# darchr/DLRM.jl

Hardware: NVIDIA B200
Metric: dlrm_train_samples_per_sec (higher is better)
Workload: dtype f32 (3xTF32 interaction forward)

## Files before the change

dlrm_jl_b200/_lib.py:

```python
from __future__ import annotations

import ctypes as C
import os
from typing import Optional

HERE = os.path.dirname(os.path.abspath(__file__))
LIB_PATH = os.path.join(HERE, "lib", "libdlrm_b200.so")

OK, EINVAL, ECUDA, ENOMEM, EOOB, ESTATE, ENCCL = 0, 1, 2, 3, 4, 5, 6
_STATUS_NAMES = {EINVAL: "DLRMB_EINVAL", ECUDA: "DLRMB_ECUDA", ENOMEM: "DLRMB_ENOMEM",
                 EOOB: "DLRMB_EOOB", ESTATE: "DLRMB_ESTATE", ENCCL: "DLRMB_ENCCL"}


class DLRMB200Error(RuntimeError):
    def __init__(self, status: int, message: str):
        super().__init__(f"{_STATUS_NAMES.get(status, status)}: {message}")
        self.status = status


_i32, _i64, _f32, _vp = C.c_int32, C.c_int64, C.c_float, C.c_void_p
_idx_args = [_vp, _i32, _i32, _i32, _i32]
_idx_mp_args = [_vp, _i32, _i32, _i32, C.POINTER(_i32)]

SIGNATURES = {
    "dlrmb_abi_version": (_i32, []),
    "dlrmb_last_error": (C.c_char_p, []),
    "dlrmb_launch_count": (_i64, []),
    "dlrmb_set_option": (_i32, [C.c_char_p, _i64]),
    "dlrmb_get_option": (_i32, [C.c_char_p, C.POINTER(_i64)]),
    "dlrmb_clock_buffer_bytes": (_i64, []),
    "dlrmb_clock_kernels": (_i32, []),
    "dlrmb_clock_enable": (_i32, [_vp]),
    "dlrmb_tables_create": (_i32, [_i32, _i32, C.POINTER(_i64), _i32, _i64, C.POINTER(_vp)]),
    "dlrmb_tables_create_ex": (_i32, [_i32, _i32, C.POINTER(_i64), _i32, _i64, _i32, C.POINTER(_vp)]),
    "dlrmb_tables_elem_bytes": (_i32, [_vp]),
    "dlrmb_tables_reserve": (_i32, [_vp, _i64]),
    "dlrmb_tables_destroy": (_i32, [_vp]),
    "dlrmb_tables_info": (_i32, [_vp, C.POINTER(_i32), C.POINTER(_i32), C.POINTER(_i64), C.POINTER(_i64)]),
    "dlrmb_tables_upload": (_i32, [_vp, _i32, _vp]),
    "dlrmb_tables_download": (_i32, [_vp, _i32, _vp]),
    "dlrmb_tables_device_ptr": (_i32, [_vp, _i32, C.POINTER(_vp)]),
    "dlrmb_tables_init_uniform": (_i32, [_vp, C.c_uint64, _vp]),
    "dlrmb_tables_sync": (_i32, [_vp]),
    "dlrmb_embedding_fwd": (_i32, [_vp, *_idx_args, _vp, _i32, _i32, _vp]),
    "dlrmb_embedding_fwd_sort": (_i32, [_vp, *_idx_args, _vp, _i32, _i32, _vp]),
    "dlrmb_interaction_fwd": (_i32, [_i32, _vp, _vp, _i32, _i32, _i32, _i32, _vp, _vp]),
    "dlrmb_interaction_bwd": (_i32, [_i32, _vp, _vp, _i32, _i32, _i32, _i32, _vp, _vp, _vp]),
    "dlrmb_embedding_sort": (_i32, [_vp, *_idx_args, _vp]),
    "dlrmb_embedding_update_sorted": (_i32, [_vp, _vp, _i32, _i32, _f32, _vp]),
    "dlrmb_embedding_bwd_sgd": (_i32, [_vp, *_idx_args, _vp, _i32, _i32, _f32, _vp]),
    "dlrmb_sort_dedup_export": (_i32, [_vp, _i32, _vp, _vp, _vp, C.POINTER(_i32)]),
    "dlrmb_check_indices": (_i32, [_vp, *_idx_args, _i32]),
    "dlrmb_bce_sigmoid_fwd_bwd": (_i32, [_i32, _vp, _vp, _i32, _vp, _vp, _vp, _vp, _vp]),
    "dlrmb_xbuf_create": (_i32, [_i32, _i64, C.POINTER(_vp)]),
    "dlrmb_xbuf_destroy": (_i32, [_vp]),
    "dlrmb_xbuf_ptr": (_i32, [_vp, C.POINTER(_vp)]),
    "dlrmb_xbuf_ipc_handle": (_i32, [_vp, _vp]),
    "dlrmb_xbuf_open": (_i32, [_i32, _vp, C.POINTER(_vp)]),
    "dlrmb_xbuf_close": (_i32, [_i32, _vp]),
    "dlrmb_tables_set_slot_map": (_i32, [_vp, C.POINTER(_i32)]),
    "dlrmb_embedding_fwd_p2p": (_i32, [_vp, *_idx_args, C.POINTER(_vp), _i32, _i32, _i32, _vp]),
    "dlrmb_embedding_fwd_p2p_sort": (_i32, [_vp, *_idx_args, C.POINTER(_vp), _i32, _i32, _i32, _vp]),
    "dlrmb_embedding_fwd_p2p_mp": (_i32, [_vp, *_idx_mp_args, C.POINTER(_vp), _i32, _i32, _i32, _vp]),
    "dlrmb_embedding_fwd_p2p_sort_mp": (_i32, [_vp, *_idx_mp_args, C.POINTER(_vp), _i32, _i32, _i32, _vp]),
    "dlrmb_peer_barrier": (_i32, [_i32, C.POINTER(_vp), _i32, _i32, _i32, _vp, _vp]),
    "dlrmb_peer_barrier_flag_bytes": (_i64, []),
    "dlrmb_peer_barrier_state_bytes": (_i64, []),
    "dlrmb_peer_allreduce_f32": (_i32, [_i32, C.POINTER(_vp), C.POINTER(_vp), _i32, _i32, _i32, _vp, _vp, _i64, _vp]),
    "dlrmb_indices_scatter_p2p": (_i32, [_i32, _vp, _i32, _i32, _i32, _i32, _vp, _i32, _vp]),
    "dlrmb_indices_scatter_p2p_mp": (_i32, [_i32, _vp, _i32, _i32, _i32, C.POINTER(_i32), _vp, _i32, _vp]),
    "dlrmb_interaction_has_warp_path": (_i32, [_i32, _i32]),
    "dlrmb_dense_fwd_bias_act": (_i32, [_i32, _vp, _vp, _i32, _i32, _i32, _vp]),
    "dlrmb_dense_bwd_scratch_floats": (_i64, [_i32]),
    "dlrmb_dense_bwd_act_bias": (_i32, [_i32, _vp, _vp, _i32, _i32, _vp, _vp, _vp, _vp]),
    "dlrmb_interaction_bwd_scatter": (_i32, [_i32, _vp, _vp, _i32, _i32, _i32, _i32, _vp, _i64, _vp, _vp]),
    "dlrmb_interaction_bwd_dx": (_i32, [_i32, _vp, _vp, _i32, _i32, _i32, _i32, _vp, _vp]),
    "dlrmb_dac_unpack": (_i32, [_i32, _vp, _i32, _vp, _vp, _vp, _vp]),
    "dlrmb_shard_plan": (_i32, [_i32, C.POINTER(_i64), _i32, C.POINTER(_i32)]),
    "dlrmb_shard_plan_mp": (_i32, [_i32, C.POINTER(_i64), C.POINTER(_i32), _i32, C.POINTER(_i32)]),
    "dlrmb_comm_unique_id": (_i32, [_vp]),
    "dlrmb_comm_create": (_i32, [_i32, _vp, _i32, _i32, C.POINTER(_vp)]),
    "dlrmb_comm_destroy": (_i32, [_vp]),
    "dlrmb_comm_info": (_i32, [_vp, C.POINTER(_i32), C.POINTER(_i32)]),
    "dlrmb_comm_a2a_indices": (_i32, [_vp, C.POINTER(_i32), _i32, _vp, _i32, _i32, _i32, _vp, _vp]),
    "dlrmb_comm_a2a_indices_mp": (_i32, [_vp, C.POINTER(_i32), _i32, _vp, _i32, _i32, C.POINTER(_i32), _vp, _vp]),
    "dlrmb_comm_a2a_fwd": (_i32, [_vp, C.POINTER(_i32), _i32, _vp, _i32, _i32, _vp, _vp]),
    "dlrmb_comm_a2a_bwd": (_i32, [_vp, C.POINTER(_i32), _i32, _vp, _i32, _i32, _vp, _vp]),
    "dlrmb_comm_allreduce_f32": (_i32, [_vp, _vp, _i64, _vp]),
    "dlrmb_comm_allgather": (_i32, [_vp, _vp, _vp, _i64, _vp]),
    "dlrmb_embedding_fwd_host": (_i32, [_vp, *_idx_args, _vp, _i32, _i32]),
    "dlrmb_interaction_fwd_host": (_i32, [_vp, _vp, _vp, _i32, _i32, _i32, _i32, _vp]),
    "dlrmb_interaction_bwd_host": (_i32, [_vp, _vp, _vp, _i32, _i32, _i32, _i32, _vp, _vp]),
    "dlrmb_embedding_bwd_sgd_host": (_i32, [_vp, *_idx_args, _vp, _i32, _i32, _f32]),
    "dlrmb_mp_max_tables": (_i32, []),
    "dlrmb_embedding_fwd_mp": (_i32, [_vp, *_idx_mp_args, _vp, _i32, _i32, _vp]),
    "dlrmb_embedding_fwd_sort_mp": (_i32, [_vp, *_idx_mp_args, _vp, _i32, _i32, _vp]),
    "dlrmb_embedding_sort_mp": (_i32, [_vp, *_idx_mp_args, _vp]),
    "dlrmb_embedding_bwd_sgd_mp": (_i32, [_vp, *_idx_mp_args, _vp, _i32, _i32, _f32, _vp]),
    "dlrmb_check_indices_mp": (_i32, [_vp, *_idx_mp_args, _i32]),
    "dlrmb_embedding_fwd_mp_host": (_i32, [_vp, *_idx_mp_args, _vp, _i32, _i32]),
    "dlrmb_embedding_bwd_sgd_mp_host": (_i32, [_vp, *_idx_mp_args, _vp, _i32, _i32, _f32]),
}

_lib: Optional[C.CDLL] = None


def load() -> C.CDLL:
    global _lib
    if _lib is not None:
        return _lib
    if not os.path.exists(LIB_PATH):
        raise DLRMB200Error(
            ESTATE,
            f"{LIB_PATH} not found: build it with `python -m dlrm_jl_b200.csrc.build` "
            "(there is no CPU or PyTorch fallback for this path)")
    lib = C.CDLL(LIB_PATH)
    for name, (res, args) in SIGNATURES.items():
        fn = getattr(lib, name)
        fn.restype = res
        fn.argtypes = args
    if lib.dlrmb_abi_version() != 1:
        raise DLRMB200Error(ESTATE, f"ABI version mismatch: library has {lib.dlrmb_abi_version()}, binding expects 1")
    _lib = lib
    return lib


def check(status: int) -> None:
# ... 18 lines not shown
```

dlrm_jl_b200/csrc/api.cu:

```cuda
#include <stdarg.h>
#include <stdlib.h>
#include <string.h>

#include <mutex>

#include "common.cuh"

namespace dlrmb {

static thread_local char tl_error[512] = "";
std::atomic<long long> g_launches{0};
Options g_opt;
static std::atomic<unsigned long long*> g_clock_buf{nullptr};
unsigned long long* clock_slot(int which) {
    unsigned long long* b = g_clock_buf.load(std::memory_order_relaxed);
    return b ? b + (size_t)which * 2 * kClockCtas : nullptr;
}

void set_error(const char* fmt, ...) {
    va_list ap;
    va_start(ap, fmt);
    vsnprintf(tl_error, sizeof(tl_error), fmt, ap);
    va_end(ap);
}
// ... 341 lines not shown
    t->sorted_B = B;
    t->sorted_P = P;
    return DLRMB_OK;
}

static int check_interaction_args(int B, int F, int d, int pad_to_mul) {
    DLRMB_REQUIRE(B > 0 && F >= 1 && d >= 1, "B, F, d must be positive (got %d, %d, %d)", B, F, d);
    DLRMB_REQUIRE(F <= 255, "F = %d exceeds 255 feature slots", F);
    DLRMB_REQUIRE(pad_to_mul >= 1, "pad_to_mul must be >= 1 (got %d)", pad_to_mul);
    return DLRMB_OK;
}

int32_t dlrmb_interaction_fwd(int32_t device, float* T, const float* x, int32_t B, int32_t F,
                              int32_t d, int32_t pad_to_mul, float* out, dlrmb_stream stream) {
    int rc = check_interaction_args(B, F, d, pad_to_mul);
    if (rc) return rc;
    DLRMB_REQUIRE(T != nullptr && out != nullptr, "T / out is null");
    DeviceGuard guard(device);
    DLRMB_REQUIRE(guard.ok, "cudaSetDevice(%d) failed", device);
    return launch_interaction_fwd(T, x, B, F, d, pad_to_mul, out, device_sm_count(device), (cudaStream_t)stream);
}

int32_t dlrmb_interaction_bwd(int32_t device, const float* dOut, const float* T, int32_t B,
                              int32_t F, int32_t d, int32_t pad_to_mul, float* dT, float* dx,
                              dlrmb_stream stream) {
    int rc = check_interaction_args(B, F, d, pad_to_mul);
    if (rc) return rc;
    DLRMB_REQUIRE(dOut && T && dT && dx, "null buffer");
    DeviceGuard guard(device);
    DLRMB_REQUIRE(guard.ok, "cudaSetDevice(%d) failed", device);
    return launch_interaction_bwd(dOut, T, B, F, d, pad_to_mul, dT, dx, device_sm_count(device), (cudaStream_t)stream);
}

int32_t dlrmb_dense_fwd_bias_act(int32_t device, float* z, const float* bias, int32_t B, int32_t N, int32_t relu,
                                 dlrmb_stream stream) {
    DLRMB_REQUIRE(B > 0 && N > 0, "B and N must be positive (got %d, %d)", B, N);
    DLRMB_REQUIRE(z && bias, "null buffer");
    DeviceGuard guard(device);
    DLRMB_REQUIRE(guard.ok, "cudaSetDevice(%d) failed", device);
    return launch_dense_fwd_bias_act(z, bias, B, N, relu, device_sm_count(device), (cudaStream_t)stream);
}

int64_t dlrmb_dense_bwd_scratch_floats(int32_t N) { return dense_bwd_scratch_floats(N); }

int32_t dlrmb_dense_bwd_act_bias(int32_t device, const float* dy, const float* y, int32_t B, int32_t N,
                                 float* dz, float* db, float* scratch, dlrmb_stream stream) {
    DLRMB_REQUIRE(B > 0 && N > 0, "B and N must be positive (got %d, %d)", B, N);
    DLRMB_REQUIRE(dy && dz && db && scratch, "null buffer");
    DeviceGuard guard(device);
    DLRMB_REQUIRE(guard.ok, "cudaSetDevice(%d) failed", device);
    return launch_dense_bwd_act_bias(dy, y, B, N, dz, db, scratch, (cudaStream_t)stream);
}

int32_t dlrmb_interaction_has_warp_path(int32_t F, int32_t d) { return interaction_has_warp_path(F, d) ? 1 : 0; }

int32_t dlrmb_interaction_bwd_scatter(int32_t device, const float* dOut, const float* T, int32_t B,
                                      int32_t F, int32_t d, int32_t pad_to_mul,
                                      const dlrmb_slot_dest* dests, int64_t sample_offset, float* dx,
                                      dlrmb_stream stream) {
    int rc = check_interaction_args(B, F, d, pad_to_mul);
    if (rc) return rc;
    DLRMB_REQUIRE(dOut && T && dests && dx, "null buffer");
    DeviceGuard guard(device);
    DLRMB_REQUIRE(guard.ok, "cudaSetDevice(%d) failed", device);
    return launch_interaction_bwd_ex(dOut, T, B, F, d, pad_to_mul, const_cast<float*>(T) , dx, dests,
                                     (long long)sample_offset, device_sm_count(device), (cudaStream_t)stream);
}

int32_t dlrmb_interaction_bwd_dx(int32_t device, const float* dOut, const float* T, int32_t B, int32_t F, int32_t d,
                                 int32_t pad_to_mul, float* dx, dlrmb_stream stream) {
    int rc = check_interaction_args(B, F, d, pad_to_mul);
    if (rc) return rc;
    DLRMB_REQUIRE(dOut && T && dx, "null buffer");
    DeviceGuard guard(device);
    DLRMB_REQUIRE(guard.ok, "cudaSetDevice(%d) failed", device);
    return launch_interaction_bwd_dx(dOut, T, B, F, d, pad_to_mul, dx, device_sm_count(device), (cudaStream_t)stream);
}

int32_t dlrmb_embedding_sort(dlrmb_tables* t, const void* idx, int32_t idx_bytes, int32_t idx_base,
                             int32_t B, int32_t P, dlrmb_stream stream) {
    GUARD(t);
    int rc = check_idx_args(t, idx, idx_bytes, idx_base, B, P);
    if (rc) return rc;
    t->sorted_valid = false;
    rc = launch_sort(t, idx, idx_bytes, idx_base, B, P, (cudaStream_t)stream);
    if (rc) return rc;
    t->sorted_valid = true;
    t->sorted_mp = false;
    t->sorted_B = B;
    t->sorted_P = P;
    return DLRMB_OK;
}

int32_t dlrmb_embedding_update_sorted(dlrmb_tables* t, const float* dT, int32_t slots,
                                      int32_t slot0, float lr, dlrmb_stream stream) {
    GUARD(t);
    if (!t->sorted_valid) {
        set_error("dlrmb_embedding_update_sorted called without a preceding dlrmb_embedding_sort");
        return DLRMB_ESTATE;
    }
    DLRMB_REQUIRE(dT != nullptr, "dT is null");
    DLRMB_REQUIRE(slot0 >= 0 && slots >= slot0 + t->ntab,
                  "slots = %d too small for slot0 = %d + %d tables", slots, slot0, t->ntab);
    return launch_update(t, dT, slots, slot0, lr, (cudaStream_t)stream);
}

// ... 346 lines not shown
```

dlrm_jl_b200/csrc/build.py:

```python
from __future__ import annotations

import os
import shutil
import subprocess
import sys

HERE = os.path.dirname(os.path.abspath(__file__))
ROOT = os.path.dirname(os.path.dirname(HERE))
LIB_DIR = os.path.join(os.path.dirname(HERE), "lib")
LIB_PATH = os.path.join(LIB_DIR, "libdlrm_b200.so")
SOURCES = ["api.cu", "lookup.cu", "interact.cu", "interact_warp.cu", "sort.cu", "update.cu", "loss.cu", "dense.cu", "p2p.cu", "loader.cu", "comm.cu"]
HEADERS = [os.path.join(HERE, "common.cuh"), os.path.join(HERE, "sort_small.cuh"), os.path.join(ROOT, "include", "dlrm_b200.h")]
NVCC_FLAGS = [
    "-gencode", "arch=compute_100a,code=sm_100a",
    "-O3", "-std=c++17", "-lineinfo",
    "-Xcompiler", "-fPIC,-O3,-Wall,-Wno-unused-function",
    "-I", os.path.join(ROOT, "include"), "-I", HERE,
]


def _nvcc() -> str:
    cand = shutil.which("nvcc") or "/usr/local/cuda/bin/nvcc"
    if not os.path.exists(cand):
        raise RuntimeError("nvcc not found: libdlrm_b200.so cannot be built")
    return cand


def needs_build() -> bool:
    if not os.path.exists(LIB_PATH):
        return True
    t = os.path.getmtime(LIB_PATH)
    deps = [os.path.join(HERE, s) for s in SOURCES] + HEADERS
    return any(os.path.getmtime(d) > t for d in deps)


def build(force: bool = False, verbose: bool = False) -> str:
    if not force and not needs_build():
        return LIB_PATH
    os.makedirs(LIB_DIR, exist_ok=True)
    obj_dir = os.path.join(LIB_DIR, "obj")
    os.makedirs(obj_dir, exist_ok=True)
    nvcc = _nvcc()
    procs = []
    objs = []
    for src in SOURCES:
        obj = os.path.join(obj_dir, src.replace(".cu", ".o"))
        objs.append(obj)
        cmd = [nvcc, *NVCC_FLAGS, "-c", os.path.join(HERE, src), "-o", obj]
        if verbose:
            cmd.insert(1, "-Xptxas=-v")
            print(" ".join(cmd), flush=True)
        procs.append((src, subprocess.Popen(cmd, stdout=subprocess.PIPE, stderr=subprocess.STDOUT, text=True)))
    failed = False
    for src, p in procs:
        out, _ = p.communicate()
        if p.returncode != 0:
            failed = True
            sys.stderr.write(f"--- nvcc failed on {src} ---\n{out}\n")
        elif verbose or out.strip():
            sys.stderr.write(out)
    if failed:
        raise RuntimeError("nvcc compilation failed")
    cmd = [nvcc, "-shared", "-o", LIB_PATH, *objs, "-gencode", "arch=compute_100a,code=sm_100a", "-lcudart", "-ldl"]
    subprocess.run(cmd, check=True)
# ... 6 lines not shown
```

dlrm_jl_b200/csrc/common.cuh:

```cuda
#pragma once
#include <cuda_bf16.h>
#include <cuda_runtime.h>
#include <stdint.h>
#include <stdio.h>
#include <string.h>

#include <type_traits>

#include <atomic>

#include "dlrm_b200.h"

namespace dlrmb {

void set_error(const char* fmt, ...);
extern std::atomic<long long> g_launches;

#define DLRMB_CUDA(expr)                                                                    \
    do {                                                                                    \
        cudaError_t _e = (expr);                                                            \
        if (_e != cudaSuccess) {                                                            \
            ::dlrmb::set_error("%s failed at %s:%d: %s", #expr, __FILE__, __LINE__,         \
                               cudaGetErrorString(_e));                                     \
            return (_e == cudaErrorMemoryAllocation) ? DLRMB_ENOMEM : DLRMB_ECUDA;          \
// ... 146 lines not shown
    uint32_t* digit_total = nullptr;
    int sorted_buf = 0;
    int64_t radix_tiles_cap = 0;
    float* partial = nullptr;
    uint8_t* tile_flags = nullptr;
    int64_t partial_tiles_cap = 0;
    uint32_t* head_list = nullptr;
    uint32_t* head_count = nullptr;
    int32_t* d_seg = nullptr;
    int64_t* d_uniq = nullptr;
    int32_t* d_nuniq = nullptr;

    bool sorted_valid = false;
    int sorted_B = 0, sorted_P = 0;
    bool sorted_mp = false;
    int32_t* h_sorted_P = nullptr;

    void* stage_idx = nullptr;  size_t stage_idx_bytes = 0;
    float* stage_a = nullptr;   size_t stage_a_bytes = 0;
    float* stage_b = nullptr;   size_t stage_b_bytes = 0;
    float* stage_c = nullptr;   size_t stage_c_bytes = 0;
    float* stage_d = nullptr;   size_t stage_d_bytes = 0;
};

namespace dlrmb {

int launch_lookup(dlrmb_tables* t, const void* idx, int idx_bytes, int idx_base, int B, int P,
                  float* out, int slots, int slot0, cudaStream_t s);
int launch_interaction_fwd(float* T, const float* x, int B, int F, int d, int pad_to_mul,
                           float* out, int sm_count, cudaStream_t s);
int launch_interaction_bwd(const float* dOut, const float* T, int B, int F, int d, int pad_to_mul,
                           float* dT, float* dx, int sm_count, cudaStream_t s);
int launch_interaction_bwd_ex(const float* dOut, const float* T, int B, int F, int d, int pad_to_mul,
                              float* dT, float* dx, const void* dests, long long sample_offset,
                              int sm_count, cudaStream_t s);
int launch_interaction_bwd_dx(const float* dOut, const float* T, int B, int F, int d, int pad_to_mul, float* dx,
                              int sm_count, cudaStream_t s);
bool interaction_has_warp_path(int F, int d);
int launch_sort(dlrmb_tables* t, const void* idx, int idx_bytes, int idx_base, int B, int P,
                cudaStream_t s);
int launch_lookup_sort(dlrmb_tables* t, const void* idx, int idx_bytes, int idx_base, int B, int P,
                       float* out, int slots, int slot0, cudaStream_t s);
int launch_update(dlrmb_tables* t, const float* dT, int slots, int slot0, float lr, cudaStream_t s);
int launch_dedup_export(dlrmb_tables* t, int k, cudaStream_t s);
int launch_init_uniform(dlrmb_tables* t, uint64_t seed, cudaStream_t s);
int launch_convert_rows(dlrmb_tables* t, int k, float* f32_buf, bool to_table, cudaStream_t s);
int launch_check_indices(dlrmb_tables* t, const void* d_idx, int idx_bytes, int idx_base, int B,
                         int P, cudaStream_t s, long long* bad_table, long long* bad_pos,
                         long long* bad_val);
int launch_bce_sigmoid(const float* z, const float* y, int B, float* prob, float* dz, float* loss,
                       float* scratch, cudaStream_t s);
int launch_dense_fwd_bias_act(float* z, const float* bias, int B, int N, int relu, int sm_count, cudaStream_t s);
int64_t dense_bwd_scratch_floats(int N);
int launch_dense_bwd_act_bias(const float* dy, const float* y, int B, int N, float* dz, float* db,
                              float* scratch, cudaStream_t s);
int launch_lookup_mp(dlrmb_tables* t, const void* idx, int idx_bytes, int idx_base, const MpGeom& g,
                     float* out, int slots, int slot0, cudaStream_t s);
int launch_lookup_sort_mp(dlrmb_tables* t, const void* idx, int idx_bytes, int idx_base, const MpGeom& g,
                          float* out, int slots, int slot0, cudaStream_t s);
int launch_sort_mp(dlrmb_tables* t, const void* idx, int idx_bytes, int idx_base, const MpGeom& g, int64_t skip_max,
                   int half, cudaStream_t s);
int sort_mp_final_half(const dlrmb_tables* t, const MpGeom& g);
int launch_update_mp(dlrmb_tables* t, const float* dT, int slots, int slot0, float lr, cudaStream_t s);
int launch_check_indices_mp(dlrmb_tables* t, const void* d_idx, int idx_bytes, int idx_base, const MpGeom& g,
                            cudaStream_t s, long long* bad_table, long long* bad_pos, long long* bad_val);
int check_mp_args(const dlrmb_tables* t, const void* idx, int idx_bytes, int idx_base, int B, const int32_t* P,
                  MpGeom* g);
void mark_sorted_mp(dlrmb_tables* t, const MpGeom& g);
int64_t lookup_grid_mp(const dlrmb_tables* t, MpGeom& g, uint32_t C, int* cshift);
static inline int64_t sorted_lookups(const dlrmb_tables* t, int k) {
    return (int64_t)t->sorted_B * (t->sorted_mp ? t->h_sorted_P[k] : t->sorted_P);
}
int device_sm_count(int device);
int64_t update_tiles_cap(int ntab, int D, int64_t max_lookups, int sm_count);
int ensure_smem_attr(const void* func, int bytes, unsigned long long* done_mask);

static inline int64_t ceil_div64(int64_t a, int64_t b) { return (a + b - 1) / b; }

}
```

dlrm_jl_b200/dense.py:

```python
from __future__ import annotations

from typing import List, Optional, Sequence

import torch
from torch import nn

from . import _lib


def _stream(t: torch.Tensor) -> int:
    return int(torch.cuda.current_stream(t.device).cuda_stream)


class _DenseFn(torch.autograd.Function):

    @staticmethod
    def forward(ctx, x: torch.Tensor, weight: torch.Tensor, bias: torch.Tensor, relu: bool,
                gw: torch.Tensor, gb: torch.Tensor, scratch: torch.Tensor):
        if not x.is_cuda:
            raise _lib.DLRMB200Error(_lib.EINVAL, "fused dense layers run on the GPU only (no CPU fallback)")
        x = x.contiguous()
        y = torch.mm(x, weight.t())
        _lib.check(_lib.load().dlrmb_dense_fwd_bias_act(
            y.device.index or 0, y.data_ptr(), bias.data_ptr(), y.shape[0], y.shape[1], 1 if relu else 0, _stream(y)))
        ctx.relu = relu
        ctx.gw, ctx.gb, ctx.scratch = gw, gb, scratch
        ctx.save_for_backward(x, weight, y if relu else None)
        return y

    @staticmethod
    def backward(ctx, dy: torch.Tensor):
        x, weight, y = ctx.saved_tensors
        dy = dy.contiguous()
        B, N = dy.shape
        dz = torch.empty_like(dy) if ctx.relu else dy
        _lib.check(_lib.load().dlrmb_dense_bwd_act_bias(
            dy.device.index or 0, dy.data_ptr(), y.data_ptr() if ctx.relu else None, B, N, dz.data_ptr(),
            ctx.gb.data_ptr(), ctx.scratch.data_ptr(), _stream(dy)))
        torch.mm(dz.t(), x, out=ctx.gw)
        dx = dz @ weight if ctx.needs_input_grad[0] else None
        return dx, None, None, None, None, None, None


class FusedDense(nn.Module):

    def __init__(self, linear: nn.Linear, relu: bool, grad_weight: Optional[torch.Tensor] = None,
                 grad_bias: Optional[torch.Tensor] = None):
        super().__init__()
        self.linear = linear
        self.relu = relu
        dev = linear.weight.device
        self.grad_weight = grad_weight if grad_weight is not None else torch.zeros_like(linear.weight)
        self.grad_bias = grad_bias if grad_bias is not None else torch.zeros_like(linear.bias)
        assert self.grad_weight.is_contiguous() and self.grad_weight.shape == linear.weight.shape
        assert self.grad_bias.is_contiguous() and self.grad_bias.shape == linear.bias.shape
        n = int(_lib.load().dlrmb_dense_bwd_scratch_floats(linear.out_features))
        self.scratch = torch.zeros(n, dtype=torch.float32, device=dev)

    def forward(self, x: torch.Tensor) -> torch.Tensor:
        return _DenseFn.apply(x, self.linear.weight, self.linear.bias, self.relu, self.grad_weight,
                              self.grad_bias, self.scratch)


class FusedMLP(nn.Module):

    def __init__(self, seq: Sequence[nn.Module], grads: Optional[Sequence[torch.Tensor]] = None):
        super().__init__()
        mods = list(seq)
        layers: List[nn.Module] = []
        gi = 0
        i = 0
        while i < len(mods):
            lin = mods[i]
            assert isinstance(lin, nn.Linear), "expected Linear (+ activation) pairs"
            act = mods[i + 1] if i + 1 < len(mods) and not isinstance(mods[i + 1], nn.Linear) else None
            gw = grads[gi] if grads is not None else None
            gb = grads[gi + 1] if grads is not None else None
            gi += 2
            layers.append(FusedDense(lin, isinstance(act, nn.ReLU), gw, gb))
            if act is not None and not isinstance(act, nn.ReLU):
                layers.append(act)
            i += 1 if act is None else 2
        self.layers = nn.Sequential(*layers)

    def forward(self, x: torch.Tensor) -> torch.Tensor:
        return self.layers(x)

    def bind_param_grads(self) -> None:
        for m in self.layers:
            if isinstance(m, FusedDense):
                m.linear.weight.grad = m.grad_weight
                m.linear.bias.grad = m.grad_bias

    def grad_buffers(self) -> List[torch.Tensor]:
        out = []
        for m in self.layers:
            if isinstance(m, FusedDense):
                out += [m.grad_weight, m.grad_bias]
        return out


__all__ = ["FusedDense", "FusedMLP"]
```

include/dlrm_b200.h:

```cpp
#ifndef DLRM_B200_H
#define DLRM_B200_H

#include <stdint.h>

#ifdef __cplusplus
extern "C" {
#endif

typedef struct dlrmb_tables dlrmb_tables;
typedef void* dlrmb_stream;

typedef enum dlrmb_status {
    DLRMB_OK = 0,
    DLRMB_EINVAL = 1,
    DLRMB_ECUDA = 2,
    DLRMB_ENOMEM = 3,
    DLRMB_EOOB = 4,
    DLRMB_ESTATE = 5,
    DLRMB_ENCCL = 6
} dlrmb_status;

#define DLRMB_ABI_VERSION 1

int32_t dlrmb_abi_version(void);
// ... 26 lines not shown

int32_t dlrmb_embedding_fwd_sort(dlrmb_tables* t, const void* idx, int32_t idx_bytes, int32_t idx_base,
                                 int32_t B, int32_t P, float* out, int32_t slots, int32_t slot0,
                                 dlrmb_stream stream);

int32_t dlrmb_interaction_fwd(int32_t device, float* T, const float* x, int32_t B, int32_t F,
                              int32_t d, int32_t pad_to_mul, float* out, dlrmb_stream stream);
int32_t dlrmb_interaction_bwd(int32_t device, const float* dOut, const float* T, int32_t B,
                              int32_t F, int32_t d, int32_t pad_to_mul, float* dT, float* dx,
                              dlrmb_stream stream);
int32_t dlrmb_interaction_has_warp_path(int32_t F, int32_t d);

int32_t dlrmb_embedding_sort(dlrmb_tables* t, const void* idx, int32_t idx_bytes, int32_t idx_base,
                             int32_t B, int32_t P, dlrmb_stream stream);
int32_t dlrmb_embedding_update_sorted(dlrmb_tables* t, const float* dT, int32_t slots,
                                      int32_t slot0, float lr, dlrmb_stream stream);
int32_t dlrmb_embedding_bwd_sgd(dlrmb_tables* t, const void* idx, int32_t idx_bytes,
                                int32_t idx_base, int32_t B, int32_t P, const float* dT,
                                int32_t slots, int32_t slot0, float lr, dlrmb_stream stream);

int32_t dlrmb_sort_dedup_export(dlrmb_tables* t, int32_t k, int64_t* uniq, int32_t* seg_offsets,
                                int32_t* perm, int32_t* n_uniq);
int32_t dlrmb_check_indices(dlrmb_tables* t, const void* idx, int32_t idx_bytes, int32_t idx_base,
                            int32_t B, int32_t P, int32_t idx_on_host);

int32_t dlrmb_mp_max_tables(void);
int32_t dlrmb_embedding_fwd_mp(dlrmb_tables* t, const void* idx, int32_t idx_bytes, int32_t idx_base, int32_t B,
                               const int32_t* P, float* out, int32_t slots, int32_t slot0, dlrmb_stream stream);
int32_t dlrmb_embedding_fwd_sort_mp(dlrmb_tables* t, const void* idx, int32_t idx_bytes, int32_t idx_base, int32_t B,
                                    const int32_t* P, float* out, int32_t slots, int32_t slot0, dlrmb_stream stream);
int32_t dlrmb_embedding_sort_mp(dlrmb_tables* t, const void* idx, int32_t idx_bytes, int32_t idx_base, int32_t B,
                                const int32_t* P, dlrmb_stream stream);
int32_t dlrmb_embedding_bwd_sgd_mp(dlrmb_tables* t, const void* idx, int32_t idx_bytes, int32_t idx_base, int32_t B,
                                   const int32_t* P, const float* dT, int32_t slots, int32_t slot0, float lr,
                                   dlrmb_stream stream);
int32_t dlrmb_check_indices_mp(dlrmb_tables* t, const void* idx, int32_t idx_bytes, int32_t idx_base, int32_t B,
                               const int32_t* P, int32_t idx_on_host);
int32_t dlrmb_embedding_fwd_mp_host(dlrmb_tables* t, const void* idx, int32_t idx_bytes, int32_t idx_base, int32_t B,
                                    const int32_t* P, float* out, int32_t slots, int32_t slot0);
int32_t dlrmb_embedding_bwd_sgd_mp_host(dlrmb_tables* t, const void* idx, int32_t idx_bytes, int32_t idx_base,
                                        int32_t B, const int32_t* P, const float* dT, int32_t slots, int32_t slot0,
                                        float lr);

int32_t dlrmb_bce_sigmoid_fwd_bwd(int32_t device, const float* logits, const float* labels, int32_t B,
                                  float* prob, float* dlogits, float* loss, float* scratch,
                                  dlrmb_stream stream);

int32_t dlrmb_dense_fwd_bias_act(int32_t device, float* z, const float* bias, int32_t B, int32_t N, int32_t relu,
                                 dlrmb_stream stream);
int64_t dlrmb_dense_bwd_scratch_floats(int32_t N);
int32_t dlrmb_dense_bwd_act_bias(int32_t device, const float* dy, const float* y, int32_t B, int32_t N,
                                 float* dz, float* db, float* scratch, dlrmb_stream stream);

int32_t dlrmb_dac_unpack(int32_t device, const void* records, int32_t B, float* labels, float* dense,
                         uint32_t* sparse, dlrmb_stream stream);

typedef struct dlrmb_xbuf dlrmb_xbuf;
int32_t dlrmb_xbuf_create(int32_t device, int64_t bytes, dlrmb_xbuf** out);
int32_t dlrmb_xbuf_destroy(dlrmb_xbuf* x);
int32_t dlrmb_xbuf_ptr(dlrmb_xbuf* x, void** dev);
int32_t dlrmb_xbuf_ipc_handle(dlrmb_xbuf* x, uint8_t* handle64);
int32_t dlrmb_xbuf_open(int32_t device, const uint8_t* handle64, void** peer_ptr);
int32_t dlrmb_xbuf_close(int32_t device, void* peer_ptr);
int32_t dlrmb_tables_set_slot_map(dlrmb_tables* t, const int32_t* slots);
int32_t dlrmb_embedding_fwd_p2p(dlrmb_tables* t, const void* idx, int32_t idx_bytes, int32_t idx_base,
                                int32_t B_global, int32_t P, float* const* peer_T, int32_t world,
                                int32_t B_local, int32_t slots, dlrmb_stream stream);

int32_t dlrmb_embedding_fwd_p2p_sort(dlrmb_tables* t, const void* idx, int32_t idx_bytes, int32_t idx_base,
                                     int32_t B_global, int32_t P, float* const* peer_T, int32_t world,
                                     int32_t B_local, int32_t slots, dlrmb_stream stream);
int32_t dlrmb_embedding_fwd_p2p_mp(dlrmb_tables* t, const void* idx, int32_t idx_bytes, int32_t idx_base,
                                   int32_t B_global, const int32_t* P, float* const* peer_T, int32_t world,
                                   int32_t B_local, int32_t slots, dlrmb_stream stream);
int32_t dlrmb_embedding_fwd_p2p_sort_mp(dlrmb_tables* t, const void* idx, int32_t idx_bytes, int32_t idx_base,
                                        int32_t B_global, const int32_t* P, float* const* peer_T, int32_t world,
                                        int32_t B_local, int32_t slots, dlrmb_stream stream);

int32_t dlrmb_peer_barrier(int32_t device, uint32_t* const* peer_flags, int32_t world, int32_t rank, int32_t channel,
                           uint32_t* state, dlrmb_stream stream);
int64_t dlrmb_peer_barrier_flag_bytes(void);
int64_t dlrmb_peer_barrier_state_bytes(void);
int32_t dlrmb_peer_allreduce_f32(int32_t device, float* const* peer_bufs, uint32_t* const* peer_flags, int32_t world,
                                 int32_t rank, int32_t channel, uint32_t* state, float* data, int64_t n,
                                 dlrmb_stream stream);
int32_t dlrmb_indices_scatter_p2p(int32_t device, const void* idx_local, int32_t idx_bytes, int32_t ntab,
                                  int32_t B_local, int32_t P, const void* const* dests_dev, int32_t rank,
                                  dlrmb_stream stream);
int32_t dlrmb_indices_scatter_p2p_mp(int32_t device, const void* idx_local, int32_t idx_bytes, int32_t ntab,
                                     int32_t B_local, const int32_t* P, const void* const* dests_dev, int32_t rank,
                                     dlrmb_stream stream);

typedef struct dlrmb_slot_dest {
    float* base;
    int64_t sample_stride;
    int64_t offset;
} dlrmb_slot_dest;
int32_t dlrmb_interaction_bwd_scatter(int32_t device, const float* dOut, const float* T, int32_t B,
                                      int32_t F, int32_t d, int32_t pad_to_mul,
                                      const dlrmb_slot_dest* dests, int64_t sample_offset, float* dx,
                                      dlrmb_stream stream);

typedef struct dlrmb_comm dlrmb_comm;
int32_t dlrmb_shard_plan(int32_t ntab, const int64_t* rows, int32_t world, int32_t* owner);
int32_t dlrmb_shard_plan_mp(int32_t ntab, const int64_t* rows, const int32_t* P, int32_t world, int32_t* owner);
int32_t dlrmb_comm_unique_id(uint8_t* id128);
// ... 34 lines not shown
```

Before: 2.335 million.

## Replace torch.mm dense layers with custom tcgen05 3xTF32 split-K GEMM

Adds a custom Blackwell GEMM that first packs both operands into hi/lo TF32 planes and then runs three tcgen05 TF32 MMAs per k-slice (3xTF32). It uses a TMA-style bulk-copy pipeline, double-buffered TMEM accumulators and split-K with an atomic last-block reduction, and fuses bias and ReLU into the epilogue. The dense-layer forward and both backward GEMMs now call it instead of torch.mm (cuBLAS FP32), with the separate bias/act pass dropped from the forward. The aim is to replace slow FP32 SIMT matmuls with tensor-core work while keeping near-FP32 accuracy. The cost is an extra pack kernel and workspace traffic per GEMM, plus the correctness risk of hand-written descriptors.

```diff
diff --git a/dlrm_jl_b200/_lib.py b/dlrm_jl_b200/_lib.py
--- a/dlrm_jl_b200/_lib.py
+++ b/dlrm_jl_b200/_lib.py
@@ -73,6 +73,8 @@
     "dlrmb_dense_fwd_bias_act": (_i32, [_i32, _vp, _vp, _i32, _i32, _i32, _vp]),
     "dlrmb_dense_bwd_scratch_floats": (_i64, [_i32]),
     "dlrmb_dense_bwd_act_bias": (_i32, [_i32, _vp, _vp, _i32, _i32, _vp, _vp, _vp, _vp]),
+    "dlrmb_gemm_f32_workspace_floats": (_i64, [_i32, _i32, _i32, _i32]),
+    "dlrmb_gemm_f32": (_i32, [_i32, _i32, _i32, _i32, _vp, _i64, _i64, _vp, _i64, _i64, _vp, _i32, _vp, _i64, _vp, _vp]),
     "dlrmb_interaction_bwd_scatter": (_i32, [_i32, _vp, _vp, _i32, _i32, _i32, _i32, _vp, _i64, _vp, _vp]),
     "dlrmb_interaction_bwd_dx": (_i32, [_i32, _vp, _vp, _i32, _i32, _i32, _i32, _vp, _vp]),
     "dlrmb_dac_unpack": (_i32, [_i32, _vp, _i32, _vp, _vp, _vp, _vp]),
diff --git a/dlrm_jl_b200/csrc/api.cu b/dlrm_jl_b200/csrc/api.cu
--- a/dlrm_jl_b200/csrc/api.cu
+++ b/dlrm_jl_b200/csrc/api.cu
@@ -417,6 +417,25 @@
     return launch_dense_bwd_act_bias(dy, y, B, N, dz, db, scratch, (cudaStream_t)stream);
 }
 
+int64_t dlrmb_gemm_f32_workspace_floats(int32_t device, int32_t M, int32_t N, int32_t K) {
+    if (M <= 0 || N <= 0 || K <= 0) return 0;
+    return gemm_workspace_floats(M, N, K, device_sm_count(device));
+}
+
+int32_t dlrmb_gemm_f32(int32_t device, int32_t M, int32_t N, int32_t K, const float* a, int64_t a_rs, int64_t a_ks,
+                       const float* b, int64_t b_rs, int64_t b_ks, const float* bias, int32_t relu, float* c,
+                       int64_t ldc, float* workspace, dlrmb_stream stream) {
+    DLRMB_REQUIRE(M > 0 && N > 0 && K > 0, "M, N and K must be positive (got %d, %d, %d)", M, N, K);
+    DLRMB_REQUIRE(a && b && c && workspace, "null buffer");
+    DLRMB_REQUIRE(a_rs >= 0 && a_ks >= 0 && b_rs >= 0 && b_ks >= 0, "negative operand stride");
+    DLRMB_REQUIRE(ldc >= N, "ldc (%lld) must be >= N (%d)", (long long)ldc, N);
+    DLRMB_REQUIRE((reinterpret_cast<uintptr_t>(workspace) & 15) == 0, "workspace must be 16-byte aligned");
+    DeviceGuard guard(device);
+    DLRMB_REQUIRE(guard.ok, "cudaSetDevice(%d) failed", device);
+    return launch_gemm_f32(M, N, K, a, a_rs, a_ks, b, b_rs, b_ks, bias, relu, c, ldc, workspace,
+                           device_sm_count(device), (cudaStream_t)stream);
+}
+
 int32_t dlrmb_interaction_has_warp_path(int32_t F, int32_t d) { return interaction_has_warp_path(F, d) ? 1 : 0; }
 
 int32_t dlrmb_interaction_bwd_scatter(int32_t device, const float* dOut, const float* T, int32_t B,
diff --git a/dlrm_jl_b200/csrc/build.py b/dlrm_jl_b200/csrc/build.py
--- a/dlrm_jl_b200/csrc/build.py
+++ b/dlrm_jl_b200/csrc/build.py
@@ -9,7 +9,7 @@
 ROOT = os.path.dirname(os.path.dirname(HERE))
 LIB_DIR = os.path.join(os.path.dirname(HERE), "lib")
 LIB_PATH = os.path.join(LIB_DIR, "libdlrm_b200.so")
-SOURCES = ["api.cu", "lookup.cu", "interact.cu", "interact_warp.cu", "sort.cu", "update.cu", "loss.cu", "dense.cu", "p2p.cu", "loader.cu", "comm.cu"]
+SOURCES = ["api.cu", "lookup.cu", "interact.cu", "interact_warp.cu", "sort.cu", "update.cu", "loss.cu", "dense.cu", "gemm.cu", "p2p.cu", "loader.cu", "comm.cu"]
 HEADERS = [os.path.join(HERE, "common.cuh"), os.path.join(HERE, "sort_small.cuh"), os.path.join(ROOT, "include", "dlrm_b200.h")]
 NVCC_FLAGS = [
     "-gencode", "arch=compute_100a,code=sm_100a",
diff --git a/dlrm_jl_b200/csrc/common.cuh b/dlrm_jl_b200/csrc/common.cuh
--- a/dlrm_jl_b200/csrc/common.cuh
+++ b/dlrm_jl_b200/csrc/common.cuh
@@ -222,6 +222,10 @@
                        float* scratch, cudaStream_t s);
 int launch_dense_fwd_bias_act(float* z, const float* bias, int B, int N, int relu, int sm_count, cudaStream_t s);
 int64_t dense_bwd_scratch_floats(int N);
+int64_t gemm_workspace_floats(int M, int N, int K, int sm_count);
+int launch_gemm_f32(int M, int N, int K, const float* a, long long a_rs, long long a_ks, const float* b,
+                    long long b_rs, long long b_ks, const float* bias, int relu, float* c, long long ldc,
+                    float* workspace, int sm_count, cudaStream_t s);
 int launch_dense_bwd_act_bias(const float* dy, const float* y, int B, int N, float* dz, float* db,
                               float* scratch, cudaStream_t s);
 int launch_lookup_mp(dlrmb_tables* t, const void* idx, int idx_bytes, int idx_base, const MpGeom& g,
diff --git a/dlrm_jl_b200/csrc/gemm.cu b/dlrm_jl_b200/csrc/gemm.cu
--- /dev/null
+++ b/dlrm_jl_b200/csrc/gemm.cu
@@ -0,0 +1,345 @@
+#include <math.h>
+
+#include "common.cuh"
+
+namespace dlrmb {
+
+constexpr int kGemmBM = 128, kGemmBN = 128, kGemmBK = 16;
+constexpr int kGemmStages = 6;
+constexpr int kGemmChunk = 32;
+constexpr int kGemmChunkKB = kGemmChunk / kGemmBK;
+constexpr int kGemmPlane = kGemmBM * kGemmBK;
+constexpr int kGemmBlock = 2 * kGemmPlane;
+constexpr int kGemmStageBytes = 2 * kGemmBlock * 4;
+constexpr int kGemmCounters = 1024;
+constexpr int kGemmThreads = 192;
+constexpr int kGemmSmem = kGemmStages * kGemmStageBytes + 1024;
+constexpr int kGemmTmemCols = 2 * kGemmBN;
+
+static_assert(kGemmBM * (kGemmBN + 1) * 4 <= kGemmStages * kGemmStageBytes, "epilogue tile reuses the ring");
+
+__device__ __forceinline__ uint32_t gsmem(const void* p) { return (uint32_t)__cvta_generic_to_shared(p); }
+
+__device__ __forceinline__ float tf32_rna(float v) {
+    uint32_t r;
+    asm("cvt.rna.tf32.f32 %0, %1;" : "=r"(r) : "f"(v));
+    return __uint_as_float(r);
+}
+
+struct PackOperand {
+    const float* src;
+    float* dst;
+    long long rs, ks;
+    int R, blocks;
+};
+__global__ void __launch_bounds__(256)
+gemm_pack_kernel(const PackOperand a, const PackOperand b, int K, int KB) {
+    __shared__ float tile[kGemmBM][kGemmBK + 1];
+    const bool is_a = blockIdx.x < (unsigned)a.blocks;
+    const int blk = is_a ? blockIdx.x : blockIdx.x - a.blocks;
+    const float* __restrict__ src = is_a ? a.src : b.src;
+    float* __restrict__ dst = is_a ? a.dst : b.dst;
+    const long long rs = is_a ? a.rs : b.rs, ks = is_a ? a.ks : b.ks;
+    const int R = is_a ? a.R : b.R;
+    const int rb = blk / KB, kb = blk % KB;
+    const int r0 = rb * kGemmBM, k0 = kb * kGemmBK;
+    const int t = threadIdx.x;
+    if (ks == 1) {
+#pragma unroll
+        for (int i = 0; i < kGemmBM * kGemmBK / 256; ++i) {
+            const int r = i * 16 + (t >> 4), k = t & 15;
+            tile[r][k] = (r0 + r < R && k0 + k < K) ? __ldg(src + (long long)(r0 + r) * rs + (k0 + k)) : 0.f;
+        }
+    } else {
+#pragma unroll
+        for (int i = 0; i < kGemmBM * kGemmBK / 256; ++i) {
+            const int idx = i * 256 + t, r = idx & (kGemmBM - 1), k = idx / kGemmBM;
+            tile[r][k] = (r0 + r < R && k0 + k < K) ? __ldg(src + (long long)(r0 + r) * rs + (long long)(k0 + k) * ks) : 0.f;
+        }
+    }
+    __syncthreads();
+    float4* head = reinterpret_cast<float4*>(dst + (size_t)blk * kGemmBlock);
+    float4* tail = head + kGemmPlane / 4;
+#pragma unroll
+    for (int i = 0; i < kGemmPlane / 4 / 256; ++i) {
+        const int q = i * 256 + t;
+        const int r = q & (kGemmBM - 1), k = (q / kGemmBM) * 4;
+        float h[4], l[4];
+#pragma unroll
+        for (int j = 0; j < 4; ++j) {
+            const float v = tile[r][k + j];
+            h[j] = tf32_rna(v);
+            l[j] = tf32_rna(v - h[j]);
+        }
+        head[q] = make_float4(h[0], h[1], h[2], h[3]);
+        tail[q] = make_float4(l[0], l[1], l[2], l[3]);
+    }
+}
+
+__device__ __forceinline__ void mbar_init(uint64_t* bar, unsigned count) {
+    asm volatile("mbarrier.init.shared::cta.b64 [%0], %1;" ::"r"(gsmem(bar)), "r"(count));
+}
+__device__ __forceinline__ void mbar_wait(uint64_t* bar, unsigned parity) {
+    uint32_t done = 0;
+    while (!done)
+        asm volatile("{\n .reg .pred p;\n mbarrier.try_wait.parity.shared::cta.b64 p, [%1], %2;\n selp.u32 %0, 1, 0, p;\n}\n"
+                     : "=r"(done) : "r"(gsmem(bar)), "r"(parity) : "memory");
+}
+__device__ __forceinline__ void mbar_arrive(uint64_t* bar) {
+    asm volatile("mbarrier.arrive.shared::cta.b64 _, [%0];" ::"r"(gsmem(bar)) : "memory");
+}
+__device__ __forceinline__ void mbar_expect_tx(uint64_t* bar, unsigned bytes) {
+    asm volatile("mbarrier.arrive.expect_tx.shared::cta.b64 _, [%0], %1;" ::"r"(gsmem(bar)), "r"(bytes) : "memory");
+}
+__device__ __forceinline__ void bulk_g2s(void* dst, const void* src, unsigned bytes, uint64_t* bar) {
+    asm volatile("cp.async.bulk.shared::cluster.global.mbarrier::complete_tx::bytes [%0], [%1], %2, [%3];"
+                 ::"r"(gsmem(dst)), "l"(src), "r"(bytes), "r"(gsmem(bar)) : "memory");
+}
+__device__ __forceinline__ void umma_commit(uint64_t* bar) {
+    asm volatile("tcgen05.commit.cta_group::1.mbarrier::arrive::one.shared::cluster.b64 [%0];" ::"r"(gsmem(bar)) : "memory");
+}
+__device__ __forceinline__ uint64_t umma_desc(uint32_t saddr) {
+    constexpr uint32_t lbo = (kGemmBM / 8) * 128, sbo = 128;
+    return (uint64_t)((saddr & 0x3FFFFu) >> 4) | ((uint64_t)(lbo >> 4) << 16) | ((uint64_t)(sbo >> 4) << 32) |
+           ((uint64_t)1 << 46);
+}
+__device__ __forceinline__ void umma_tf32(uint32_t d_tmem, uint64_t a, uint64_t b, uint32_t acc) {
+    constexpr uint32_t idesc = (1u << 4) | (2u << 7) | (2u << 10) | ((uint32_t)(kGemmBN >> 3) << 17) |
+                               ((uint32_t)(kGemmBM >> 4) << 24);
+    asm volatile(
+        "{\n .reg .pred p;\n setp.ne.b32 p, %4, 0;\n"
+        " tcgen05.mma.cta_group::1.kind::tf32 [%0], %1, %2, %3, p;\n}\n"
+        ::"r"(d_tmem), "l"(a), "l"(b), "r"(idesc), "r"(acc) : "memory");
+}
+__device__ __forceinline__ void epi_sync() { asm volatile("bar.sync 1, 128;" ::: "memory"); }
+
+struct GemmArgs {
+    const float* a;
+    const float* b;
+    const float* bias;
+    float* c;
+    long long ldc;
+    float* partial;
+    unsigned* counters;
+    int M, N, KB, splits, relu;
+};
+
+__global__ void __launch_bounds__(kGemmThreads, 1)
+gemm_tf32x3_kernel(const GemmArgs p) {
+    extern __shared__ uint8_t smem_raw[];
+    uint8_t* smem = reinterpret_cast<uint8_t*>((reinterpret_cast<uintptr_t>(smem_raw) + 1023) & ~uintptr_t(1023));
+    __shared__ __align__(8) uint64_t full[kGemmStages], empty[kGemmStages], accf[2], acce[2];
+    __shared__ uint32_t tmem_base;
+    __shared__ int is_last;
+    const int warp = threadIdx.x >> 5, lane = threadIdx.x & 31;
+    const int mb = blockIdx.x, nb = blockIdx.y, split = blockIdx.z;
+    const int kb0 = (int)((long long)split * p.KB / p.splits), kb1 = (int)((long long)(split + 1) * p.KB / p.splits);
+    const int nk = kb1 - kb0;
+    const int nchunks = (nk + kGemmChunkKB - 1) / kGemmChunkKB;
+
+    if (threadIdx.x == 0) {
+        for (int s = 0; s < kGemmStages; ++s) { mbar_init(&full[s], 1); mbar_init(&empty[s], 1); }
+        for (int b = 0; b < 2; ++b) { mbar_init(&accf[b], 1); mbar_init(&acce[b], 128); }
+        asm volatile("fence.mbarrier_init.release.cluster;" ::: "memory");
+    }
+    if (warp == 5) {
+        asm volatile("tcgen05.alloc.cta_group::1.sync.aligned.shared::cta.b32 [%0], %1;" ::"r"(gsmem(&tmem_base)), "r"(kGemmTmemCols));
+        asm volatile("tcgen05.relinquish_alloc_permit.cta_group::1.sync.aligned;");
+    }
+    asm volatile("tcgen05.fence::before_thread_sync;" ::: "memory");
+    __syncthreads();
+    asm volatile("tcgen05.fence::after_thread_sync;" ::: "memory");
+    const uint32_t tmem = tmem_base;
+
+    if (warp == 4) {
+        if (lane == 0) {
+            const float* ga = p.a + ((size_t)mb * p.KB + kb0) * kGemmBlock;
+            const float* gb = p.b + ((size_t)nb * p.KB + kb0) * kGemmBlock;
+            for (int it = 0; it < nk; ++it) {
+                const int s = it % kGemmStages;
+                mbar_wait(&empty[s], ((it / kGemmStages) & 1) ^ 1);
+                uint8_t* st = smem + (size_t)s * kGemmStageBytes;
+                mbar_expect_tx(&full[s], kGemmStageBytes);
+                bulk_g2s(st, ga + (size_t)it * kGemmBlock, kGemmBlock * 4, &full[s]);
+                bulk_g2s(st + kGemmBlock * 4, gb + (size_t)it * kGemmBlock, kGemmBlock * 4, &full[s]);
+            }
+        }
+    } else if (warp == 5) {
+        if (lane == 0) {
+            for (int it = 0; it < nk; ++it) {
+                const int s = it % kGemmStages, c = it / kGemmChunkKB, buf = c & 1;
+                const bool first = (it % kGemmChunkKB) == 0;
+                if (first) {
+                    mbar_wait(&acce[buf], ((c >> 1) & 1) ^ 1);
+                    asm volatile("tcgen05.fence::after_thread_sync;" ::: "memory");
+                }
+                mbar_wait(&full[s], (it / kGemmStages) & 1);
+                asm volatile("tcgen05.fence::after_thread_sync;" ::: "memory");
+                const uint32_t sa = gsmem(smem + (size_t)s * kGemmStageBytes);
+                const uint32_t sb = sa + kGemmBlock * 4;
+                const uint32_t d = tmem + (uint32_t)(buf * kGemmBN);
+#pragma unroll
+                for (int j = 0; j < kGemmBK / 8; ++j) {
+                    const uint32_t off = (uint32_t)j * 2 * (kGemmBM / 8) * 128;
+                    const uint64_t ah = umma_desc(sa + off), at = umma_desc(sa + kGemmPlane * 4 + off);
+                    const uint64_t bh = umma_desc(sb + off), bt = umma_desc(sb + kGemmPlane * 4 + off);
+                    umma_tf32(d, at, bh, (first && j == 0) ? 0u : 1u);
+                    umma_tf32(d, ah, bt, 1u);
+                    umma_tf32(d, ah, bh, 1u);
+                }
+                umma_commit(&empty[s]);
+                if ((it % kGemmChunkKB) == kGemmChunkKB - 1 || it == nk - 1) umma_commit(&accf[buf]);
+            }
+        }
+    } else {
+        float acc[kGemmBN];
+#pragma unroll
+        for (int j = 0; j < kGemmBN; ++j) acc[j] = 0.f;
+        const uint32_t lane_addr = tmem + ((uint32_t)(warp * 32) << 16);
+        for (int c = 0; c < nchunks; ++c) {
+            const int buf = c & 1;
+            mbar_wait(&accf[buf], (c >> 1) & 1);
+            asm volatile("tcgen05.fence::after_thread_sync;" ::: "memory");
+#pragma unroll
+            for (int g = 0; g < kGemmBN / 32; ++g) {
+                uint32_t v[32];
+#pragma unroll
+                for (int h = 0; h < 4; ++h)
+                    asm volatile("tcgen05.ld.sync.aligned.32x32b.x8.b32 {%0,%1,%2,%3,%4,%5,%6,%7}, [%8];"
+                                 : "=r"(v[8 * h + 0]), "=r"(v[8 * h + 1]), "=r"(v[8 * h + 2]), "=r"(v[8 * h + 3]),
+                                   "=r"(v[8 * h + 4]), "=r"(v[8 * h + 5]), "=r"(v[8 * h + 6]), "=r"(v[8 * h + 7])
+                                 : "r"(lane_addr + (uint32_t)(buf * kGemmBN + g * 32 + 8 * h)));
+                asm volatile("tcgen05.wait::ld.sync.aligned;" ::: "memory");
+#pragma unroll
+                for (int j = 0; j < 32; ++j) acc[g * 32 + j] = __fadd_rn(acc[g * 32 + j], __uint_as_float(v[j]));
+            }
+            asm volatile("tcgen05.fence::before_thread_sync;" ::: "memory");
+            mbar_arrive(&acce[buf]);
+        }
+        float* tile = reinterpret_cast<float*>(smem);
+        constexpr int TP = kGemmBN + 1;
+        const int row = warp * 32 + lane;
+#pragma unroll
+        for (int j = 0; j < kGemmBN; ++j) tile[row * TP + j] = acc[j];
+        __syncwarp();
+        const int m0 = mb * kGemmBM, n0 = nb * kGemmBN;
+        const int tiles = gridDim.x * gridDim.y, tile_id = nb * gridDim.x + mb;
+        bool write_c = true;
+        if (p.splits > 1) {
+            const int mrows = min(kGemmBM, p.M - m0), ncols = min(kGemmBN, p.N - n0);
+            float* part = p.partial + ((size_t)split * tiles + tile_id) * (kGemmBM * kGemmBN);
+            for (int rr = 0; rr < 32; ++rr) {
+                const int r = warp * 32 + rr;
+                if (r >= mrows) break;
+#pragma unroll
+                for (int q = 0; q < kGemmBN / 32; ++q)
+                    if (q * 32 + lane < ncols) part[r * kGemmBN + q * 32 + lane] = tile[r * TP + q * 32 + lane];
+            }
+            __threadfence();
+            epi_sync();
+            if (threadIdx.x == 0) {
+                is_last = (atomicAdd(p.counters + tile_id, 1u) == (unsigned)(p.splits - 1));
+                __threadfence();
+            }
+            epi_sync();
+            write_c = is_last != 0;
+            if (write_c) {
+                const bool col_ok = 4 * lane < ncols;
+                for (int z = 0; z < p.splits; ++z) {
+                    const float4* src = reinterpret_cast<const float4*>(
+                        p.partial + ((size_t)z * tiles + tile_id) * (kGemmBM * kGemmBN) + (size_t)(warp * 32) * kGemmBN);
+                    float4 v[32];
+#pragma unroll
+                    for (int rr = 0; rr < 32; ++rr)
+                        v[rr] = (col_ok && warp * 32 + rr < mrows) ? __ldcg(src + rr * (kGemmBN / 4) + lane) : make_float4(0.f, 0.f, 0.f, 0.f);
+#pragma unroll
+                    for (int rr = 0; rr < 32; ++rr) {
+                        float* t = tile + (warp * 32 + rr) * TP + 4 * lane;
+                        const float w[4] = {v[rr].x, v[rr].y, v[rr].z, v[rr].w};
+#pragma unroll
+                        for (int j = 0; j < 4; ++j) t[j] = z == 0 ? w[j] : t[j] + w[j];
+                    }
+                }
+                if (threadIdx.x == 0) p.counters[tile_id] = 0;
+            }
+        }
+        if (write_c) {
+#pragma unroll
+            for (int q = 0; q < kGemmBN / 32; ++q) {
+                const int col = n0 + q * 32 + lane;
+                if (col >= p.N) continue;
+                const float bv = p.bias ? __ldg(p.bias + col) : 0.f;
+                for (int rr = 0; rr < 32; ++rr) {
+                    const int r = warp * 32 + rr;
+                    if (m0 + r >= p.M) break;
+                    float v = tile[r * TP + q * 32 + lane];
+                    if (p.bias) v += bv;
+                    if (p.relu) v = fmaxf(v, 0.f);
+                    p.c[(long long)(m0 + r) * p.ldc + col] = v;
+                }
+            }
+        }
+    }
+    asm volatile("tcgen05.fence::before_thread_sync;" ::: "memory");
+    __syncthreads();
+    if (warp == 5) {
+        asm volatile("tcgen05.fence::after_thread_sync;" ::: "memory");
+        asm volatile("tcgen05.dealloc.cta_group::1.sync.aligned.b32 %0, %1;" ::"r"(tmem), "r"(kGemmTmemCols));
+    }
+}
+
+static inline int64_t pack_floats(int R, int K) {
+    return ceil_div64(R, kGemmBM) * ceil_div64(K, kGemmBK) * kGemmBlock;
+}
+
+static inline int gemm_splits(int M, int N, int K, int sm_count) {
+    const int64_t tiles = ceil_div64(M, kGemmBM) * ceil_div64(N, kGemmBN);
+    const int64_t kb = ceil_div64(K, kGemmBK);
+    if (tiles >= sm_count || tiles > kGemmCounters) return 1;
+    int64_t s = sm_count / tiles;
+    const int64_t by_k = kb / kGemmChunkKB;
+    const int64_t by_sum = (int64_t)sqrt(3.0 * (double)kb / 8.0);
+    if (s > by_k) s = by_k;
+    if (s > by_sum) s = by_sum;
+    return s < 1 ? 1 : (int)s;
+}
+
+int64_t gemm_workspace_floats(int M, int N, int K, int sm_count) {
+    const int splits = gemm_splits(M, N, K, sm_count);
+    const int64_t tiles = ceil_div64(M, kGemmBM) * ceil_div64(N, kGemmBN);
+    return kGemmCounters + pack_floats(M, K) + pack_floats(N, K) +
+           (splits > 1 ? (int64_t)splits * tiles * kGemmBM * kGemmBN : 0);
+}
+
+int launch_gemm_f32(int M, int N, int K, const float* a, long long a_rs, long long a_ks, const float* b,
+                    long long b_rs, long long b_ks, const float* bias, int relu, float* c, long long ldc,
+                    float* workspace, int sm_count, cudaStream_t s) {
+    static unsigned long long attr_done = 0;
+    int rc = ensure_smem_attr((const void*)gemm_tf32x3_kernel, kGemmSmem, &attr_done);
+    if (rc) return rc;
+    const int KB = (int)ceil_div64(K, kGemmBK);
+    const int MB = (int)ceil_div64(M, kGemmBM), NB = (int)ceil_div64(N, kGemmBN);
+    float* pa = workspace + kGemmCounters;
+    float* pb = pa + pack_floats(M, K);
+    const PackOperand opa = {a, pa, a_rs, a_ks, M, MB * KB}, opb = {b, pb, b_rs, b_ks, N, NB * KB};
+    gemm_pack_kernel<<<(unsigned)(opa.blocks + opb.blocks), 256, 0, s>>>(opa, opb, K, KB);
+    DLRMB_LAUNCH_CHECK();
+    GemmArgs p;
+    p.a = pa;
+    p.b = pb;
+    p.bias = bias;
+    p.c = c;
+    p.ldc = ldc;
+    p.partial = pb + pack_floats(N, K);
+    p.counters = reinterpret_cast<unsigned*>(workspace);
+    p.M = M;
+    p.N = N;
+    p.KB = KB;
+    p.splits = gemm_splits(M, N, K, sm_count);
+    p.relu = relu;
+    gemm_tf32x3_kernel<<<dim3((unsigned)MB, (unsigned)NB, (unsigned)p.splits), kGemmThreads, kGemmSmem, s>>>(p);
+    DLRMB_LAUNCH_CHECK();
+    return DLRMB_OK;
+}
+
+}
diff --git a/dlrm_jl_b200/dense.py b/dlrm_jl_b200/dense.py
--- a/dlrm_jl_b200/dense.py
+++ b/dlrm_jl_b200/dense.py
@@ -12,19 +12,28 @@
     return int(torch.cuda.current_stream(t.device).cuda_stream)
 
 
+def _gemm(x_dev: int, M: int, N: int, K: int, a: torch.Tensor, a_rs: int, a_ks: int, b: torch.Tensor, b_rs: int,
+          b_ks: int, bias: Optional[torch.Tensor], relu: bool, c: torch.Tensor, ws: torch.Tensor, stream: int) -> None:
+    _lib.check(_lib.load().dlrmb_gemm_f32(
+        x_dev, M, N, K, a.data_ptr(), a_rs, a_ks, b.data_ptr(), b_rs, b_ks,
+        bias.data_ptr() if bias is not None else None, 1 if relu else 0, c.data_ptr(), c.stride(0), ws.data_ptr(), stream))
+
+
 class _DenseFn(torch.autograd.Function):
 
     @staticmethod
     def forward(ctx, x: torch.Tensor, weight: torch.Tensor, bias: torch.Tensor, relu: bool,
-                gw: torch.Tensor, gb: torch.Tensor, scratch: torch.Tensor):
+                gw: torch.Tensor, gb: torch.Tensor, scratch: torch.Tensor, layer: "FusedDense"):
         if not x.is_cuda:
             raise _lib.DLRMB200Error(_lib.EINVAL, "fused dense layers run on the GPU only (no CPU fallback)")
         x = x.contiguous()
-        y = torch.mm(x, weight.t())
-        _lib.check(_lib.load().dlrmb_dense_fwd_bias_act(
-            y.device.index or 0, y.data_ptr(), bias.data_ptr(), y.shape[0], y.shape[1], 1 if relu else 0, _stream(y)))
+        B, n_in = x.shape
+        n_out = weight.shape[0]
+        y = torch.empty((B, n_out), dtype=torch.float32, device=x.device)
+        ws = layer.workspace(B)
+        _gemm(x.device.index or 0, B, n_out, n_in, x, n_in, 1, weight, n_in, 1, bias, relu, y, ws, _stream(y))
         ctx.relu = relu
-        ctx.gw, ctx.gb, ctx.scratch = gw, gb, scratch
+        ctx.gw, ctx.gb, ctx.scratch, ctx.ws = gw, gb, scratch, ws
         ctx.save_for_backward(x, weight, y if relu else None)
         return y
 
@@ -33,13 +42,18 @@
         x, weight, y = ctx.saved_tensors
         dy = dy.contiguous()
         B, N = dy.shape
+        n_in = x.shape[1]
+        dev, st = dy.device.index or 0, _stream(dy)
         dz = torch.empty_like(dy) if ctx.relu else dy
         _lib.check(_lib.load().dlrmb_dense_bwd_act_bias(
-            dy.device.index or 0, dy.data_ptr(), y.data_ptr() if ctx.relu else None, B, N, dz.data_ptr(),
-            ctx.gb.data_ptr(), ctx.scratch.data_ptr(), _stream(dy)))
-        torch.mm(dz.t(), x, out=ctx.gw)
-        dx = dz @ weight if ctx.needs_input_grad[0] else None
-        return dx, None, None, None, None, None, None
+            dev, dy.data_ptr(), y.data_ptr() if ctx.relu else None, B, N, dz.data_ptr(),
+            ctx.gb.data_ptr(), ctx.scratch.data_ptr(), st))
+        dx = None
+        if ctx.needs_input_grad[0]:
+            dx = torch.empty((B, n_in), dtype=torch.float32, device=dy.device)
+            _gemm(dev, B, n_in, N, dz, N, 1, weight, 1, n_in, None, False, dx, ctx.ws, st)
+        _gemm(dev, N, n_in, B, dz, 1, N, x, 1, n_in, None, False, ctx.gw, ctx.ws, st)
+        return dx, None, None, None, None, None, None, None
 
 
 class FusedDense(nn.Module):
@@ -56,10 +70,21 @@
         assert self.grad_bias.is_contiguous() and self.grad_bias.shape == linear.bias.shape
         n = int(_lib.load().dlrmb_dense_bwd_scratch_floats(linear.out_features))
         self.scratch = torch.zeros(n, dtype=torch.float32, device=dev)
+        self._ws: Optional[torch.Tensor] = None
+
+    def workspace(self, B: int) -> torch.Tensor:
+        lib = _lib.load()
+        dev = self.linear.weight.device
+        i, o = self.linear.in_features, self.linear.out_features
+        n = max(int(lib.dlrmb_gemm_f32_workspace_floats(dev.index or 0, M, N, K))
+                for M, N, K in ((B, o, i), (B, i, o), (o, i, B)))
+        if self._ws is None or self._ws.numel() < n:
+            self._ws = torch.zeros(n, dtype=torch.float32, device=dev)
+        return self._ws
 
     def forward(self, x: torch.Tensor) -> torch.Tensor:
         return _DenseFn.apply(x, self.linear.weight, self.linear.bias, self.relu, self.grad_weight,
-                              self.grad_bias, self.scratch)
+                              self.grad_bias, self.scratch, self)
 
 
 class FusedMLP(nn.Module):
diff --git a/include/dlrm_b200.h b/include/dlrm_b200.h
--- a/include/dlrm_b200.h
+++ b/include/dlrm_b200.h
@@ -102,6 +102,11 @@
 int32_t dlrmb_dense_bwd_act_bias(int32_t device, const float* dy, const float* y, int32_t B, int32_t N,
                                  float* dz, float* db, float* scratch, dlrmb_stream stream);
 
+int64_t dlrmb_gemm_f32_workspace_floats(int32_t device, int32_t M, int32_t N, int32_t K);
+int32_t dlrmb_gemm_f32(int32_t device, int32_t M, int32_t N, int32_t K, const float* a, int64_t a_rs, int64_t a_ks,
+                       const float* b, int64_t b_rs, int64_t b_ks, const float* bias, int32_t relu, float* c,
+                       int64_t ldc, float* workspace, dlrmb_stream stream);
+
 int32_t dlrmb_dac_unpack(int32_t device, const void* records, int32_t B, float* labels, float* dense,
                          uint32_t* sparse, dlrmb_stream stream);
 
```

After: 2.332 million (median of 6 runs). Within noise of the previous version (-0.1%).
